# Exawind/hypre-mini-app

Measured on AMD Instinct MI355X. Metric: GMRES+AMG solve GDOF/s (N_global*iterations/t_solve; iterations/sec in iterations_per_s), 512^3 Laplacian, higher is better.
Workload: dtype f64

## Files before the change

### hypre-mini-app_amd/csrc/amg_solve.cpp

```cpp
#include <algorithm>
#include <cmath>

#include "amg.hpp"
#include "kernels.hpp"
#include "profile.hpp"
#include "solvers.hpp"

namespace mi {

bool &zero_guess_hint() {
  static bool hint = false;
  return hint;
}

static int g_zero_skip = -1;
int zero_skip_mode() {
  if (g_zero_skip < 0) {
    const char *e = getenv("MI_HYPRE_GS_ZERO_SKIP");
    g_zero_skip = e ? std::max(0, std::min(3, atoi(e))) : 3;
  }
  return g_zero_skip;
}
void set_zero_skip_mode(int mode) { g_zero_skip = std::max(0, std::min(3, mode)); }

// ... 523 lines not shown
  AmgLevel &L0 = L[0];
  const bool permuted = !L0.perm.empty();
  if (permuted)
    k::gather(f, L0.d_perm.p, L0.f.p, L0.n, s);
  else
    k::copy(f, L0.f.p, L0.n, s);
  if (zero_guess) {
    if (!zero_cycle_ignores_u(0)) k::fill(L0.u.p, L0.n, 0.0, s);
  } else if (permuted)
    k::gather(e, L0.d_perm.p, L0.u.p, L0.n, s);
  else
    k::copy(e, L0.u.p, L0.n, s);
  cycle(0, zero_guess);
  if (permuted)
    k::scatter_set(e, L0.d_perm.p, L0.u.p, L0.n, s);
  else
    k::copy(L0.u.p, e, L0.n, s);
}

void BoomerAMG::solve(ParCSR &A, ParVector &b, ParVector &x) {
  if (!is_setup) setup(A);
  if (!L.empty() && source_matrix && L[0].A == source_matrix && L[0].A->assembly_stamp != source_stamp)
    fail(1, "BoomerAMGSolve: the values of the matrix changed (IJMatrix update round) after this solver was set up on it "
            "and its first level is that matrix itself; call HYPRE_BoomerAMGSetup again");
  MI_REQUIRE(x.ncomp == b.ncomp, "BoomerAMGSolve: b and x differ in their number of components");
  MI_REQUIRE(x.n == L[0].n && b.n == L[0].n, "BoomerAMGSolve: vector size does not match the matrix");
  Comm &comm = my_comm();
  hipStream_t s = ctx().stream;
  AmgLevel &L0 = L[0];
  const bool permuted = !L0.perm.empty();
  const int n = L0.n, nc = b.ncomp;
  int it = 0;
  double rel = 0.0, bn = 0.0;
  if (p.tol > 0.0) bn = std::sqrt(par_dot_host(comm, b.all(), b.all(), b.len(), s));
  const bool zero_first = zero_guess_hint();
  zero_guess_hint() = false;
  while (it < p.max_iter) {
    const bool zero = zero_first && it == 0;
    for (int c = 0; c < nc; c++) {
      const double *bc = b.all() + (size_t)c * (size_t)n;
      double *xc = x.all() + (size_t)c * (size_t)n;
      if (it == 0 || nc > 1) {
        if (permuted)
          k::gather(bc, L0.d_perm.p, L0.f.p, n, s);
        else
          k::copy(bc, L0.f.p, n, s);
      }
      if (zero) {
        if (!zero_cycle_ignores_u(0)) k::fill(L0.u.p, n, 0.0, s);
      } else if (permuted)
        k::gather(xc, L0.d_perm.p, L0.u.p, n, s);
      else
        k::copy(xc, L0.u.p, n, s);
      cycle(0, zero);
      if (permuted)
        k::scatter_set(xc, L0.d_perm.p, L0.u.p, n, s);
      else
        k::copy(L0.u.p, xc, n, s);
    }
    it++;
    if (p.tol > 0.0) {
      double rr = 0.0;
      for (int c = 0; c < nc; c++) {
        const size_t o = (size_t)c * (size_t)n;
        A.matvec(comm, -1.0, x.all() + o, 1.0, b.all() + o, L0.tmp.p, s);
        rr += par_dot_host(comm, L0.tmp.p, L0.tmp.p, n, s);
      }
      const double rn = std::sqrt(rr);
      rel = (bn > 0.0) ? rn / bn : rn;
      if (p.print_level > 1 && comm.rank == 0) printf("    BoomerAMG cycle %3d   ||r||/||b|| = %e\n", it, rel);
      if (rel <= p.tol) break;
    }
  }
  num_iterations = it;
  final_rel_res = rel;
}

}
```

### hypre-mini-app_amd/csrc/capi.cpp

```cpp
#include <limits>
#include <algorithm>
#include <cmath>
#include <cstring>
#include <thread>

#include "HYPRE_mi_ext.h"
#include "_hypre_parcsr_ls.h"
#include "ij_assembly.hpp"
#include "kernels.hpp"
#include "profile.hpp"
#include "solvers.hpp"
#include "amg_setup_internal.hpp"

using namespace mi;

namespace {

int g_error_flag = 0;
std::string g_last_error;

int record_error(int code, const std::string &msg) {
  g_error_flag |= code;
  g_last_error = msg;
  fprintf(stderr, "mi_hypre error (%d): %s\n", code, msg.c_str());
// ... 1832 lines not shown
  API_END
}
HYPRE_Int HYPRE_MI_GetCounter(const char *name, long long *value) {
  API_BEGIN
  const std::string n(name ? name : "");
  if (n == "pool_cached_bytes" || n == "pool_hits" || n == "pool_misses") {
    long long cb = 0, h = 0, m = 0;
    dev_pool_stats(&cb, &h, &m);
    *value = n == "pool_cached_bytes" ? cb : n == "pool_hits" ? h : m;
    return 0;
  }
  if (n.rfind("arena_", 0) == 0) {
    long long mp = 0, iu = 0, pm = 0, pu = 0;
    dev_arena_stats(&mp, &iu, &pm, &pu);
    if (n == "arena_mapped_bytes") *value = mp;
    else if (n == "arena_in_use_bytes") *value = iu;
    else if (n == "arena_peak_mapped_bytes") *value = pm;
    else if (n == "arena_peak_in_use_bytes") *value = pu;
    else fail(HYPRE_ERROR_ARG, "GetCounter: unknown counter " + n);
    return 0;
  }
  if (n == "ij_device_assemblies")
    *value = ij::counters().device_assemblies;
  else if (n == "ij_value_updates")
    *value = ij::counters().value_updates;
  else if (n == "ij_device_value_updates")
    *value = ij::counters().device_value_updates;
  else if (n == "ij_update_kernels_us" || n == "ij_update_dictionary_us" || n == "ij_update_mirror_us")
    *value = (long long)(1e6 * (n == "ij_update_kernels_us" ? ij::counters().t_update_kernels
                                : n == "ij_update_dictionary_us" ? ij::counters().t_update_dict : ij::counters().t_update_mirror));
  else if (n == "ij_entries_fetched_to_host")
    *value = ij::counters().entries_fetched;
  else if (n == "ij_host_mirror_bytes")
    *value = ij::counters().host_mirror_bytes;
  else if (n == "ij_device_sort_lds_capacity")
    *value = ij::SORT_LDS_CAP;
  else if (n == "ij_last_kernels_us" || n == "ij_last_mirror_us" || n == "ij_last_format_us")
    *value = (long long)(1e6 * (n == "ij_last_kernels_us" ? ij::counters().t_kernels
                                : n == "ij_last_mirror_us" ? ij::counters().t_mirror : ij::counters().t_format));
  else if (n == "matvec_overlapped")
    *value = ctx().n_matvec_overlapped;
  else if (n == "gs_overlapped")
    *value = ctx().n_gs_overlapped;
  else if (n == "gs_in_order")
    *value = ctx().n_gs_in_order;
  else if (n == "allreduce")
    *value = ctx().n_allreduce;
  else if (n == "halo_exchange")
    *value = ctx().n_halo_exchange;
  else if (n == "allgather")
    *value = ctx().n_allgather;
  else if (n == "value_storage_row_mapped")
    *value = ctx().n_value_row_mapped;
  else if (setup_reuse_counter(n.c_str()) >= 0)
    *value = setup_reuse_counter(n.c_str());
  else if (dist_setup_counter(n.c_str()) >= 0)
    *value = dist_setup_counter(n.c_str());
  else
    fail(HYPRE_ERROR_ARG, "GetCounter: unknown counter " + n);
  API_END
}
HYPRE_Int HYPRE_MI_SetZeroGuessMode(HYPRE_Int mode) {
  API_BEGIN
  if (mode < 0 || mode > 3) fail(HYPRE_ERROR_ARG, "SetZeroGuessMode: 0..3");
  set_zero_skip_mode(mode);
  API_END
}
HYPRE_Int HYPRE_MI_BoomerAMGPoisonWorkVectors(HYPRE_Solver solver) {
  API_BEGIN
  BoomerAMG &a = AMG(solver)->amg;
  const double nan = std::numeric_limits<double>::quiet_NaN();
  hipStream_t s = ctx().stream;
  for (BoomerAMG *h = &a; h; h = h->tail.get())
    for (AmgLevel &Lv : h->L) {
      if (Lv.u.p && Lv.n) k::fill(Lv.u.p, Lv.n, nan, s);
      if (Lv.tmp.p && Lv.n) k::fill(Lv.tmp.p, Lv.n, nan, s);
      if (Lv.snap.p && Lv.n) k::fill(Lv.snap.p, Lv.n, nan, s);
    }
  MI_HIP(hipStreamSynchronize(s));
  API_END
}
HYPRE_Int HYPRE_MI_TileScheduleCheck(HYPRE_Int n, const HYPRE_BigInt *row_ptr, HYPRE_Int row_cap, HYPRE_Int tile_entries,
                                     HYPRE_Int *ntiles, HYPRE_Int *mismatch) {
  API_BEGIN
  ensure_init();
  MI_REQUIRE(n >= 0 && row_ptr && mismatch, "TileScheduleCheck: arguments");
  MI_REQUIRE(tile_entries == k::SPMV_TILE || tile_entries == k::SPMV_TILE_WIDE, "TileScheduleCheck: tile_entries is 2048 or 4096");
  static_assert(sizeof(HYPRE_BigInt) == sizeof(long long), "row pointer width");
  bool aligned_h = true, aligned_d = true;
  const std::vector<int> host = k::build_row_blocks((int)n, reinterpret_cast<const int64_t *>(row_ptr), &aligned_h, (int)row_cap,
                                                    (int)tile_entries);
  DVec<long long> ia((size_t)n + 1);
  MI_HIP(hipMemcpy(ia.p, row_ptr, ((size_t)n + 1) * sizeof(long long), hipMemcpyHostToDevice));
  DVec<int> rb;
  std::vector<int> dev;
  sk::tile_schedule_device((int)n, ia.p, (int)row_cap, (int)tile_entries, rb, dev, aligned_d, ctx().stream);
  if (ntiles) *ntiles = (HYPRE_Int)host.size() - 1;
  *mismatch = 0;
  const size_t m = std::min(host.size(), dev.size());
  for (size_t t = 0; t < m && !*mismatch; t++)
    if (host[t] != dev[t]) *mismatch = (HYPRE_Int)t + 1;
  if (!*mismatch && host.size() != dev.size()) *mismatch = (HYPRE_Int)m + 1;
  if (!*mismatch && aligned_h != aligned_d) *mismatch = (HYPRE_Int)m + 2;
  API_END
}

// ... 82 lines not shown
    unsigned long long res[3];
    differing(b, res);
    if (res[0])
      fail(HYPRE_ERROR_GENERIC, "arena self-test: a live block was overwritten: " + std::to_string(res[0]) + " of " + std::to_string(b.n) +
                                    " bytes differ, first at " + std::to_string(res[1]) + ", last at " + std::to_string(res[2]) +
                                    "; block at arena offset " + std::to_string((unsigned long long)(b.p - (unsigned char *)nullptr) & 0xffffffffffull));
    dev_free(b.p);
    cur -= b.n;
    ok++;
  };
  for (int r = 0; r < rounds; r++) {
    const unsigned long long v = rnd();
    const bool grow = live.empty() || (v & 3) != 0 || live.size() < 8;
    if (grow && live.size() < 4096) {
      const int bits = 1 + (int)(rnd() % 34);
      size_t n = (size_t)(rnd() & ((1ull << bits) - 1)) + 1;
      n = std::min<size_t>(n, (size_t)std::max<HYPRE_BigInt>(1, max_block_bytes));
      Blk b{(unsigned char *)dev_alloc(n), n, (unsigned char)(1 + (rnd() % 250))};
      for (const Blk &o : live)
        if (b.p < o.p + o.n && o.p < b.p + b.n)
          fail(HYPRE_ERROR_GENERIC, "arena self-test: the allocator handed out a block that intersects a live one (round " +
                                        std::to_string(r) + ", " + std::to_string(n) + " bytes)");
      if (getenv("MI_ARENA_TEST_OWN_FILL"))
        k::fill_bytes(b.p, n, b.tag, s);
      else
        MI_HIP(hipMemsetAsync(b.p, b.tag, n, s));
      if (getenv("MI_ARENA_TEST_VERIFY_FILL")) {
        unsigned long long res[3];
        differing(b, res);
        if (res[0])
          fail(HYPRE_ERROR_GENERIC, "arena self-test: the fill of a fresh block is incomplete: " + std::to_string(res[0]) + " of " +
                                        std::to_string(n) + " bytes, first " + std::to_string(res[1]) + ", last " + std::to_string(res[2]));
      }
      live.push_back(b);
      cur += n;
      peak = std::max(peak, cur);
    } else {
      check_and_free((size_t)(rnd() % live.size()));
    }
    if ((r & 255) == 255 && !getenv("MI_ARENA_TEST_NO_TRIM")) dev_pool_trim();
  }
  MI_HIP(hipStreamSynchronize(s));
  while (!live.empty()) check_and_free(live.size() - 1);
  dev_pool_trim();
  if (verified) *verified = ok;
  if (peak_bytes) *peak_bytes = (HYPRE_BigInt)peak;
  API_END
}
HYPRE_Int HYPRE_MI_SetValueDictionary(HYPRE_Int on) {
  API_BEGIN
  k::set_value_dictionary(on != 0);
  API_END
}
HYPRE_Int HYPRE_MI_GetGSChunk(HYPRE_Int *rows) {
  *rows = ctx().gs_chunk;
  return 0;
}
HYPRE_Int HYPRE_MI_KrylovGetResidualHistory(HYPRE_Solver solver, HYPRE_Real *norms, HYPRE_Int max_n, HYPRE_Int *n) {
  API_BEGIN
  KrylovSolver *kk = KR(solver);
  const int m = std::min<int>(max_n, (int)kk->norms.size());
  for (int i = 0; i < m; i++) norms[i] = kk->norms[(size_t)i];
  if (n) *n = (int)kk->norms.size();
  API_END
}
HYPRE_Int HYPRE_MI_KrylovGetSolveSeconds(HYPRE_Solver solver, HYPRE_Real *seconds) {
  API_BEGIN
  *seconds = KR(solver)->solve_seconds;
  API_END
}
HYPRE_Int HYPRE_MI_BoomerAMGGetNumLevels(HYPRE_Solver solver, HYPRE_Int *n) {
  API_BEGIN
  *n = (HYPRE_Int)AMG(solver)->amg.total_levels();
  API_END
}
HYPRE_Int HYPRE_MI_BoomerAMGGetOperatorComplexity(HYPRE_Solver solver, HYPRE_Real *cx) {
  API_BEGIN
  *cx = AMG(solver)->amg.operator_complexity();
  API_END
}
HYPRE_Int HYPRE_MI_BoomerAMGGetSetupSeconds(HYPRE_Solver solver, HYPRE_Real *seconds) {
  API_BEGIN
  *seconds = AMG(solver)->amg.setup_seconds;
  API_END
}
static AmgLevel &level_ref(AmgSolver *a, int level, BoomerAMG **owner = nullptr, int *local = nullptr) {
  if (level < 0 || level >= a->amg.total_levels()) fail(HYPRE_ERROR_ARG, "AMG level out of range");
  int loc = 0;
  BoomerAMG &o = a->amg.owner_of(level, loc);
  if (owner) *owner = &o;
  if (local) *local = loc;
  return o.L[(size_t)loc];
}
static const HostCSR &level_csr(AmgSolver *a, int level, int which) {
  BoomerAMG *o = nullptr;
  int loc = 0;
  AmgLevel &L = level_ref(a, level, &o, &loc);
  o->ensure_host(loc);
  switch (which) {
    case 0: return L.A->diag;
    case 1: return L.A->offd;
    case 2:
    case 3:
    case 4:
    case 5: {
      const ParCSR *M = (which == 2 || which == 4) ? L.Pm.get() : L.Rm.get();
// ... 507 lines not shown
```

### hypre-mini-app_amd/csrc/krylov.cpp

```cpp
#include <cmath>
#include <cstring>

#include "HYPRE_parcsr_ls.h"
#include "kernels.hpp"
#include "solvers.hpp"

extern "C" const char *HYPRE_MI_LastErrorMessage(void);

namespace mi {

void KrylovSolver::run_precond_setup(ParCSR &A, ParVector &b, ParVector &x) {
  if (!precond_setup) return;
  const int rc = precond_setup(precond_data, &A, &b, &x);
  if (rc) fail(rc, std::string("preconditioner setup failed: ") + HYPRE_MI_LastErrorMessage());
}


void KrylovSolver::apply_precond(ParCSR &A, ParVector &rhs, ParVector &out) {
  hipStream_t s = ctx().stream;
  if (precond_solve) {
    k::fill(out.all(), out.len(), 0.0, s);
    zero_guess_hint() = true;
    precond_solve(precond_data, &A, &rhs, &out);
    zero_guess_hint() = false;
  } else {
    k::copy(rhs.all(), out.all(), out.len(), s);
  }
}

void KrylovSolver::matvec_all(ParCSR &A, double alpha, const double *x, double beta, const double *b, double *y, int nloc,
                              int ncomp, int prof) {
  Comm &comm = current_comm();
  hipStream_t s = ctx().stream;
  for (int c = 0; c < ncomp; c++) {
    const size_t o = (size_t)c * (size_t)nloc;
    A.matvec(comm, alpha, x + o, beta, b ? b + o : nullptr, y + o, s, prof);
  }
}

BoomerAMG *KrylovSolver::amg_in_level_order(ParCSR &A, int n) const {
  static const bool enabled = !(getenv("MI_HYPRE_GMRES_PERMUTED") && atoi(getenv("MI_HYPRE_GMRES_PERMUTED")) == 0);
  if (!enabled || !precond_data) return nullptr;
  if (precond_solve != reinterpret_cast<ParSolverFcn>(&HYPRE_BoomerAMGSolve)) return nullptr;
  SolverBase *sb = static_cast<SolverBase *>(precond_data);
  if (sb->kind != SolverBase::K_AMG) return nullptr;
  BoomerAMG &amg = static_cast<AmgSolver *>(sb)->amg;
  if (!amg.is_setup || amg.p.max_iter != 1 || amg.p.tol != 0.0 || amg.L.empty()) return nullptr;
  AmgLevel &L0 = amg.L[0];
  if (L0.perm.empty() || L0.A == &A || L0.n != n || !L0.A->on_device) return nullptr;
  if (amg.source_matrix != &A || amg.source_stamp != A.assembly_stamp) return nullptr;
  return &amg;
}

BoomerAMG *KrylovSolver::enter_level_order(ParCSR &A_in, ParVector &b_in, ParVector &x_in, ParCSR *&A, ParVector *&b,
                                           ParVector *&x) {
  const int n = b_in.n, nc = b_in.ncomp;
  BoomerAMG *amg = amg_in_level_order(A_in, n);
  A = &A_in;
  b = &b_in;
  x = &x_in;
  if (!amg) return nullptr;
  hipStream_t s = ctx().stream;
  if (bp.n != n || bp.ncomp != nc) {
    bp.init(b_in.start, b_in.end, nc);
    xp.init(b_in.start, b_in.end, nc);
  }
  for (int c = 0; c < nc; c++) {
    const size_t o = (size_t)c * (size_t)n;
    k::gather(b_in.all() + o, amg->L[0].d_perm.p, bp.all() + o, n, s);
    k::gather(x_in.all() + o, amg->L[0].d_perm.p, xp.all() + o, n, s);
  }
  A = amg->L[0].A;
  b = &bp;
  x = &xp;
  return amg;
}

void KrylovSolver::leave_level_order(BoomerAMG *amg, ParVector &x_in) {
  if (!amg) return;
  for (int c = 0; c < x_in.ncomp; c++) {
    const size_t o = (size_t)c * (size_t)x_in.n;
    k::scatter_set(x_in.all() + o, amg->L[0].d_perm.p, xp.all() + o, x_in.n, ctx().stream);
  }
}

const double *KrylovSolver::precond_in_order(BoomerAMG *amg, ParCSR &A, ParVector &rhs, ParVector &out, bool need_copy) {
  if (!amg) {
    apply_precond(A, rhs, out);
    return out.all();
  }
  hipStream_t s = ctx().stream;
  AmgLevel &L0 = amg->L[0];
  const int n = L0.n, nc = rhs.ncomp;
  double *own_f = L0.f.p;
  for (int c = 0; c < nc; c++) {
    const size_t o = (size_t)c * (size_t)n;
    L0.f.p = rhs.all() + o;
    if (!amg->zero_cycle_ignores_u(0)) k::fill(L0.u.p, n, 0.0, s);
    try {
      amg->cycle(0, true);
    } catch (...) {
      L0.f.p = own_f;
      throw;
    }
    L0.f.p = own_f;
    if (nc == 1 && !need_copy) return L0.u.p;
    k::copy(L0.u.p, out.all() + o, n, s);
  }
  return out.all();
}

void GmresSolver::setup(ParCSR &A, ParVector &b, ParVector &x) {
  ensure_init();
  MI_REQUIRE(b.ncomp == x.ncomp, "GMRES: b and x differ in their number of components");
  r.init(b.start, b.end, b.ncomp);
  w.init(b.start, b.end, b.ncomp);
  if (!p.empty() && (p[0]->n != b.n || p[0]->ncomp != b.ncomp || p[0]->start != b.start)) p.clear();
  if (!z.empty() && (z[0]->n != b.n || z[0]->ncomp != b.ncomp || z[0]->start != b.start)) z.clear();
  run_precond_setup(A, b, x);
}

int GmresSolver::solve(ParCSR &A_in, ParVector &b_in, ParVector &x_in) {
  TraceRange trace_solve(flexible ? "mi_hypre FlexGMRESSolve" : (ortho ? "mi_hypre COGMRESSolve" : "mi_hypre GMRESSolve"));
  ensure_init();
  Ctx &c = ctx();
  Comm &comm = current_comm();
  hipStream_t s = c.stream;
  const double t_start = wall_time();
  const int nloc = b_in.n, nc = b_in.ncomp;
  const int n = nloc * nc;
  MI_REQUIRE(x_in.ncomp == nc && x_in.n == nloc, "GMRES: b and x differ in size");
  const int kd = k_dim < 1 ? 1 : k_dim;
  MI_REQUIRE(kd + 2 <= (ortho > 1 ? 120 : 250), "GMRES: k_dim too large for the device scalar slots");
  MI_REQUIRE(ortho >= 0 && ortho <= 2, "GMRES: orthogonalisation must be 0 (MGS), 1 or 2 (classical passes)");
  if (r.n != nloc || r.ncomp != nc) setup(A_in, b_in, x_in);
  const double epsmac = 1.e-16;
  auto basis = [&](int i) -> ParVector & {
    while ((int)p.size() <= i) {
      std::unique_ptr<ParVector> v(new ParVector());
      v->init(b_in.start, b_in.end, nc);
      p.push_back(std::move(v));
    }
    return *p[(size_t)i];
  };
  auto zvec = [&](int i) -> ParVector & {
    while ((int)z.size() <= i) {
      std::unique_ptr<ParVector> v(new ParVector());
      v->init(b_in.start, b_in.end, nc);
      z.push_back(std::move(v));
    }
    return *z[(size_t)i];
  };
  std::vector<double> cs((size_t)kd + 1, 0.0), sn((size_t)kd + 1, 0.0), rs((size_t)kd + 1, 0.0);
  std::vector<std::vector<double>> hh((size_t)kd + 1, std::vector<double>((size_t)kd, 0.0));
  double *slots = c.red_out.p;

  ParCSR *Ap;
  ParVector *bq, *xq;
  BoomerAMG *amg = enter_level_order(A_in, b_in, x_in, Ap, bq, xq);
  ParCSR &A = *Ap;
  ParVector &b = *bq;
  ParVector &x = *xq;
  auto precond = [&](ParVector &rhs, ParVector &out, bool need_copy) -> const double * {
    return precond_in_order(amg, A, rhs, out, need_copy);
  };

  auto mv = [&](double alpha, const double *xv, double beta, const double *bv, double *yv) {
    matvec_all(A, alpha, xv, beta, bv, yv, nloc, nc, k::PROF_SPMV_L0);
  };
  static const bool poll = !(getenv("MI_HYPRE_GMRES_POLL") && atoi(getenv("MI_HYPRE_GMRES_POLL")) == 0);
  auto fetch_column = [&](const double *norm_slot, double *vec, int count) {
    if (!poll || count > 255) {
      k::scale_inv_sqrt_dev(norm_slot, vec, n, s);
      MI_HIP(hipMemcpyAsync(c.h_pinned, slots, (size_t)count * sizeof(double), hipMemcpyDeviceToHost, s));
      MI_HIP(hipStreamSynchronize(s));
      return;
    }
    const unsigned long long seq = ++c.post_seq;
    k::scale_inv_sqrt_post(norm_slot, vec, n, slots, count, c.h_pinned + 256, c.h_post_flag, seq, s);
    const double t0 = wall_time();
    unsigned spins = 0;
    while (__atomic_load_n(c.h_post_flag, __ATOMIC_ACQUIRE) != seq) {
      if ((++spins & 0xffffu) == 0 && wall_time() - t0 > 30.0) {
        MI_HIP(hipStreamSynchronize(s));
        if (__atomic_load_n(c.h_post_flag, __ATOMIC_ACQUIRE) != seq) fail(1, "GMRES: the Hessenberg column was not posted");
        break;
      }
    }
    memcpy(c.h_pinned, c.h_pinned + 256, (size_t)count * sizeof(double));
  };
  ParVector &p0 = basis(0);
  mv(-1.0, x.all(), 1.0, b.all(), p0.data());
  const double b_norm = std::sqrt(par_dot_host(comm, b.all(), b.all(), n, s));
  double r_norm = std::sqrt(par_dot_host(comm, p0.data(), p0.data(), n, s));
  const double r_norm_0 = r_norm;
  const double den = (b_norm > 0.0) ? b_norm : r_norm;
  const double eps = std::max(atol, tol * den);
  int iter = 0;
  converged = false;
  norms.clear();
  norms.push_back(r_norm);
  const bool chatty = print_level > 1 && comm.rank == 0;
  bool nan_seen = (b_norm != b_norm) || (r_norm != r_norm);
  if (nan_seen && comm.rank == 0 && print_level > 0)
    printf("ERROR detected by mi_hypre GMRES: NaN in the right-hand side, the initial guess or the operator\n");
  if (chatty) {
    printf("=============================================\n\n");
    printf("Iters     resid.norm     conv.rate  rel.res.norm\n");
    printf("-----    ------------    ---------- ------------\n");
  }

  while (iter < max_iter && !nan_seen) {
    rs[0] = r_norm;
    if (r_norm == 0.0) {
      converged = true;
      break;
    }
    if (r_norm <= eps && iter >= min_iter) {
      mv(-1.0, x.all(), 1.0, b.all(), r.data());
      r_norm = std::sqrt(par_dot_host(comm, r.data(), r.data(), n, s));
      if (r_norm <= eps) {
        converged = true;
        break;
      }
      if (chatty) printf("false convergence 1\n");
    }
    k::scale(1.0 / r_norm, basis(0).data(), n, s);
    int i = 0;
    while (i < kd && iter < max_iter) {
      i++;
      iter++;
      ParVector &pi = basis(i);
      ParVector &pim1 = basis(i - 1);
      ParVector &dir = flexible ? zvec(i - 1) : r;
      const double *mp;
      {
        TraceRange tr("precond (BoomerAMG cycle)");
        mp = precond(pim1, dir, flexible);
      }
      mv(1.0, mp, 0.0, nullptr, pi.data());
      TraceRange trace_ortho("Gram-Schmidt + Givens");
      if (ortho == 0) {
        par_dot(comm, basis(0).data(), pi.data(), n, slots, s);
        for (int j = 1; j <= i; j++) {
          k::axpy_dot(slots + j - 1, -1.0, basis(j - 1).data(), pi.data(), j < i ? basis(j).data() : nullptr, n,
                      slots + j, s);
          if (comm.size > 1) comm.allreduce_dev(slots + j, 1, CommDType::F64, CommOp::SUM, s), c.n_allreduce++;
        }
        fetch_column(slots + i, pi.data(), i + 1);
        for (int j = 0; j < i; j++) hh[(size_t)j][(size_t)i - 1] = c.h_pinned[j];
      } else {
        std::vector<const double *> vecs((size_t)i);
        for (int j = 0; j < i; j++) vecs[(size_t)j] = basis(j).data();
        for (int q = 0; q < ortho; q++) {
          double *cs_dev = slots + 128 * q;
          k::mass_dot(vecs.data(), i, pi.data(), n, cs_dev, s);
          if (comm.size > 1) comm.allreduce_dev(cs_dev, (size_t)i, CommDType::F64, CommOp::SUM, s), c.n_allreduce++;
          k::mass_axpy(vecs.data(), i, cs_dev, -1.0, pi.data(), n, s);
        }
        double *nrm = (ortho == 1) ? slots + i : slots + 128 + i;
        par_dot(comm, pi.data(), pi.data(), n, nrm, s);
        fetch_column(nrm, pi.data(), 128 * (ortho - 1) + i + 1);
        for (int j = 0; j < i; j++) {
          double hsum = c.h_pinned[j];
          if (ortho > 1) hsum += c.h_pinned[128 + j];
          hh[(size_t)j][(size_t)i - 1] = hsum;
        }
        c.h_pinned[i] = c.h_pinned[128 * (ortho - 1) + i];
      }
      const double t = std::sqrt(c.h_pinned[i] > 0.0 ? c.h_pinned[i] : 0.0);
      hh[(size_t)i][(size_t)i - 1] = t;
      for (int j = 1; j < i; j++) {
        const double tt = hh[(size_t)j - 1][(size_t)i - 1];
        hh[(size_t)j - 1][(size_t)i - 1] = sn[(size_t)j - 1] * hh[(size_t)j][(size_t)i - 1] + cs[(size_t)j - 1] * tt;
        hh[(size_t)j][(size_t)i - 1] = -sn[(size_t)j - 1] * tt + cs[(size_t)j - 1] * hh[(size_t)j][(size_t)i - 1];
      }
      double gamma = std::sqrt(hh[(size_t)i - 1][(size_t)i - 1] * hh[(size_t)i - 1][(size_t)i - 1] +
                               hh[(size_t)i][(size_t)i - 1] * hh[(size_t)i][(size_t)i - 1]);
      if (gamma == 0.0) gamma = epsmac;
      cs[(size_t)i - 1] = hh[(size_t)i - 1][(size_t)i - 1] / gamma;
      sn[(size_t)i - 1] = hh[(size_t)i][(size_t)i - 1] / gamma;
      rs[(size_t)i] = -hh[(size_t)i][(size_t)i - 1] * rs[(size_t)i - 1];
      rs[(size_t)i] /= gamma;
      rs[(size_t)i - 1] = cs[(size_t)i - 1] * rs[(size_t)i - 1];
      hh[(size_t)i - 1][(size_t)i - 1] =
          sn[(size_t)i - 1] * hh[(size_t)i][(size_t)i - 1] + cs[(size_t)i - 1] * hh[(size_t)i - 1][(size_t)i - 1];
      const double prev = r_norm;
      r_norm = std::fabs(rs[(size_t)i]);
      norms.push_back(r_norm);
      if (chatty)
        printf("% 5d    %e    %f   %e\n", iter, r_norm, prev > 0 ? r_norm / prev : 0.0,
               b_norm > 0 ? r_norm / b_norm : r_norm);
      if (r_norm != r_norm) {
        nan_seen = true;
        break;
      }
      if (r_norm <= eps && iter >= min_iter) break;
    }
    if (nan_seen) break;
    std::vector<double> y(rs.begin(), rs.begin() + i);
    y[(size_t)i - 1] = y[(size_t)i - 1] / hh[(size_t)i - 1][(size_t)i - 1];
    for (int kk = i - 2; kk >= 0; kk--) {
      double t = 0.0;
      for (int j = kk + 1; j < i; j++) t -= hh[(size_t)kk][(size_t)j] * y[(size_t)j];
      t += y[(size_t)kk];
      y[(size_t)kk] = t / hh[(size_t)kk][(size_t)kk];
    }
    if (flexible) {
      for (int j = i - 1; j >= 0; j--) k::axpy(y[(size_t)j], zvec(j).data(), x.all(), n, s);
    } else {
      {
        std::vector<const double *> vp((size_t)i);
        std::vector<double> cf((size_t)i);
        for (int j = i - 1, q = 0; j >= 0; j--, q++) {
          vp[(size_t)q] = basis(j).data();
          cf[(size_t)q] = y[(size_t)j];
        }
        k::lin_comb(vp.data(), cf.data(), i, true, w.data(), n, s);
      }
      const double *mw = precond(w, r, false);
      k::axpy(1.0, mw, x.all(), n, s);
    }
    if (r_norm <= eps && iter >= min_iter) {
      mv(-1.0, x.all(), 1.0, b.all(), r.data());
      r_norm = std::sqrt(par_dot_host(comm, r.data(), r.data(), n, s));
      if (r_norm <= eps) {
        converged = true;
        break;
      }
      if (chatty) printf("false convergence 2\n");
      k::copy(r.data(), basis(0).data(), n, s);
      i = 0;
    }
    if (flexible) {
      if (i) {
        mv(-1.0, x.all(), 1.0, b.all(), basis(0).data());
        r_norm = std::sqrt(par_dot_host(comm, basis(0).data(), basis(0).data(), n, s));
      }
      continue;
    }
    for (int j = i; j > 0; j--) {
      rs[(size_t)j - 1] = -sn[(size_t)j - 1] * rs[(size_t)j];
      rs[(size_t)j] = cs[(size_t)j - 1] * rs[(size_t)j];
    }
    if (i) {
      std::vector<const double *> vp;
      std::vector<double> cf;
      for (int j = i; j > 0; j--) {
        vp.push_back(basis(j).data());
        cf.push_back(rs[(size_t)j]);
      }
      k::lin_comb(vp.data(), cf.data(), (int)vp.size(), true, basis(i).data(), n, s);
      const double *v0[2] = {basis(0).data(), basis(i).data()};
      const double c0[2] = {rs[0], 1.0};
      k::lin_comb(v0, c0, 2, true, basis(0).data(), n, s);
    }
  }
  leave_level_order(amg, x_in);
  MI_HIP(hipStreamSynchronize(s));
  num_iterations = iter;
  rel_residual_norm = (b_norm > 0.0) ? r_norm / b_norm : r_norm;
  solve_seconds = wall_time() - t_start;
// ... 208 lines not shown
```

### hypre-mini-app_amd/csrc/mi_internal.hpp

```cpp
#pragma once

#include <hip/hip_runtime.h>

#include <cstdint>
#include <cstdio>
#include <cstdlib>
#include <functional>
#include <memory>
#include <stdexcept>
#include <string>
#include <type_traits>
#include <vector>

namespace mi {

using gidx = long long;

struct Error : std::runtime_error {
  int code;
  Error(int c, const std::string &m) : std::runtime_error(m), code(c) {}
};

[[noreturn]] inline void fail(int code, const std::string &msg) { throw Error(code, msg); }

// ... 195 lines not shown
  virtual ~Comm() {}
  virtual const char *name() const = 0;
  virtual void allreduce_dev(void *buf, size_t count, CommDType t, CommOp op, hipStream_t s) = 0;
  virtual void exchange_dev(const std::vector<PeerBuf> &sends, const std::vector<PeerBuf> &recvs, hipStream_t s) = 0;
  virtual void allgather_dev(const void *send, void *recv, size_t bytes_per_rank, hipStream_t s) = 0;
  virtual void allreduce_host(void *buf, size_t count, CommDType t, CommOp op);
  virtual void allgather_host(const void *send, void *recv, size_t bytes_per_rank);
  virtual void exchange_host_fixed(const std::vector<PeerBuf> &sends, const std::vector<PeerBuf> &recvs);
  void exchange_host(const std::vector<int> &peers_send, const std::vector<std::vector<char>> &send,
                     std::vector<int> &peers_recv, std::vector<std::vector<char>> &recv);
  void allgatherv_host(const void *mine, size_t bytes, std::vector<size_t> &offs, std::vector<char> &out);
  virtual bool host_transport() const { return false; }
  void barrier();
};

std::unique_ptr<Comm> make_self_comm();
std::unique_ptr<Comm> make_rccl_comm(const void *unique_id, int rank, int size);
void rccl_get_unique_id(void *out128);

struct CommCallbacks {
  void *ctx;
  void (*allreduce)(void *ctx, void *buf, size_t count, int dtype, int op);
  void (*allgather)(void *ctx, const void *send, void *recv, size_t bytes_per_rank);
  void (*exchange)(void *ctx, int nsend, const int *send_peers, void *const *send_ptrs, const size_t *send_bytes,
                   int nrecv, const int *recv_peers, void *const *recv_ptrs, const size_t *recv_bytes);
};
std::unique_ptr<Comm> make_callback_comm(const CommCallbacks &cb, int rank, int size);
std::unique_ptr<Comm> make_ipc_exchange_comm(std::unique_ptr<Comm> &inner, size_t slot_bytes);
bool comm_check_transport_error(Comm &c, hipStream_t s);
int comm_transport_verdict(Comm &c, hipStream_t s);
std::unique_ptr<Comm> make_comm_from_env();

struct KernelTimer;

struct Ctx {
  bool inited = false;
  int device = 0;
  hipStream_t stream = nullptr;
  hipStream_t comm_stream = nullptr;
  hipEvent_t ev_packed = nullptr, ev_halo = nullptr;
  std::unique_ptr<Comm> comm;
  DVec<double> red_partials;
  DVec<double> red_out;
  DVec<unsigned> red_ticket;
  double *h_pinned = nullptr;
  unsigned long long *h_post_flag = nullptr;
  unsigned long long post_seq = 0;
  int gs_chunk = 8;
  int verbose = 0;
  KernelTimer *timer = nullptr;
  long long n_matvec_overlapped = 0, n_gs_overlapped = 0, n_gs_in_order = 0;
  long long n_allreduce = 0, n_halo_exchange = 0, n_allgather = 0;
  long long n_value_row_mapped = 0;
};
Ctx &ctx();
void ensure_init();
void zero_on_stream(void *p, size_t bytes);
Comm &current_comm();

struct TraceRange {
  explicit TraceRange(const char *name);
  ~TraceRange();
  TraceRange(const TraceRange &) = delete;
  TraceRange &operator=(const TraceRange &) = delete;
  bool on = false;
};

void parallel_for(int64_t n, const std::function<void(int64_t, int64_t, int)> &fn, int max_threads = 0);
int host_threads();
double wall_time();

}
```

### hypre-mini-app_amd/csrc/solvers.hpp

```cpp
#pragma once
#include "amg.hpp"

namespace mi {

struct SolverBase {
  enum Kind { K_GMRES, K_BICGSTAB, K_PCG, K_AMG, K_ILU, K_FSAI } kind;
  explicit SolverBase(Kind k) : kind(k) {}
  virtual ~SolverBase() {}
};

typedef int (*ParSolverFcn)(void *, void *, void *, void *);

struct AmgSolver : SolverBase {
  BoomerAMG amg;
  AmgSolver() : SolverBase(K_AMG) {}
};

struct KrylovSolver : SolverBase {
  double tol = 1e-6, atol = 0.0;
  int max_iter = 1000, min_iter = 0, k_dim = 5, print_level = 0, logging = 0;
  ParSolverFcn precond_solve = nullptr, precond_setup = nullptr;
  void run_precond_setup(ParCSR &A, ParVector &b, ParVector &x);
  void *precond_data = nullptr;
  int num_iterations = 0;
  double rel_residual_norm = 0.0;
  bool converged = false;
  std::vector<double> norms;
  double solve_seconds = 0.0;
  explicit KrylovSolver(Kind k) : SolverBase(k) {}
  void apply_precond(ParCSR &A, ParVector &rhs, ParVector &out);
  void matvec_all(ParCSR &A, double alpha, const double *x, double beta, const double *b, double *y, int nloc, int ncomp,
                  int prof);
  BoomerAMG *amg_in_level_order(ParCSR &A, int n) const;
  ParVector bp, xp;
  BoomerAMG *enter_level_order(ParCSR &A_in, ParVector &b_in, ParVector &x_in, ParCSR *&A, ParVector *&b, ParVector *&x);
  void leave_level_order(BoomerAMG *amg, ParVector &x_in);
  const double *precond_in_order(BoomerAMG *amg, ParCSR &A, ParVector &rhs, ParVector &out, bool need_copy);
};

struct GmresSolver : KrylovSolver {
  std::vector<std::unique_ptr<ParVector>> p;
  bool flexible = false;
  int ortho = 0;
  std::vector<std::unique_ptr<ParVector>> z;
  ParVector r, w;
  GmresSolver() : KrylovSolver(K_GMRES) {}
  void setup(ParCSR &A, ParVector &b, ParVector &x);
  int solve(ParCSR &A, ParVector &b, ParVector &x);
};

struct BicgstabSolver : KrylovSolver {
  ParVector r0, r, pv, v, q, sv, t;
  BicgstabSolver() : KrylovSolver(K_BICGSTAB) {}
  void setup(ParCSR &A, ParVector &b, ParVector &x);
  int solve(ParCSR &A, ParVector &b, ParVector &x);
};

struct PcgSolver : KrylovSolver {
  ParVector r, pv, sv;
  int two_norm = 0;
  PcgSolver() : KrylovSolver(K_PCG) {}
  void setup(ParCSR &A, ParVector &b, ParVector &x);
  int solve(ParCSR &A, ParVector &b, ParVector &x);
};

struct IluSolver : SolverBase {
  int ilu_type = 0, level_of_fill = 0, max_iter = 20, print_level = 0, tri_solve = 1, lower_it = 5, upper_it = 5;
  double tol = 1e-7;
  int iter_type = 0, iter_option = 0, iter_max_iter = 100;
  double iter_tol = 1e-3;
  int iter_sweeps = 0;
  double iter_correction = -1.0, iter_residual = -1.0;
  std::vector<double> iter_corr_hist, iter_res_hist;
  bool is_setup = false, levels_built = false;
  int n = 0;
  sk::DCsr LU;
  DVec<long long> dpos;
  DVec<int> order_l, order_u;
  std::vector<int> lptr, uptr;
  DVec<double> y, t, r, z;
  DVec<double> rall;
  int num_iterations = 0;
  double final_rel_res = 0.0;
  IluSolver() : SolverBase(K_ILU) {}
  void setup(ParCSR &A, Comm &comm);
  void iterative_factor(Comm &comm, long long row0);
  void apply(const double *rhs, double *out);
  int solve(ParCSR &A, ParVector &b, ParVector &x);
};

struct FsaiSolver : SolverBase {
// ... 33 lines not shown
```

### hypre-mini-app_amd/mi_hypre.py

```python
import ctypes as C
import os

import numpy as np

_HERE = os.path.dirname(os.path.abspath(__file__))
LIB_PATH = os.environ.get("MI_HYPRE_LIB") or os.path.join(_HERE, "libmi_hypre.so")

HYPRE_PARCSR = 5555
HYPRE_MEMORY_DEVICE = 1
HYPRE_EXEC_DEVICE = 1
HYPRE_ERROR_GENERIC = 1
HYPRE_ERROR_CONV = 256

c_big = C.c_longlong
c_int = C.c_int
c_dbl = C.c_double
vp = C.c_void_p

PROF_SPMV_L0, PROF_RELAX_L0, PROF_DOT, PROF_AXPY = 0, 1, 2, 3
PROF_LEVELS = 16
PROF_LVL_RESID, PROF_LVL_RELAX, PROF_LVL_RESTRICT, PROF_LVL_PROLONG = 4, 4 + 16, 4 + 32, 4 + 48
PROF_LVL_RELAX0 = 4 + 64

ALLREDUCE_FN = C.CFUNCTYPE(None, vp, vp, C.c_size_t, c_int, c_int)
# ... 707 lines not shown


def laplace3d(nx, ny, nz, stencil, ilower, iupper):
    nnz = c_big()
    rows, cols, vals, rhs = vp(), vp(), vp(), vp()
    call("HYPRE_MI_Laplace3D", nx, ny, nz, stencil, c_big(ilower), c_big(iupper), C.byref(nnz), C.byref(rows),
         C.byref(cols), C.byref(vals), C.byref(rhs))
    return dict(nnz=nnz.value, rows=rows.value, cols=cols.value, vals=vals.value, rhs=rhs.value,
                nloc=iupper - ilower + 1)


def laplace3d_free(g):
    for k in ("rows", "cols", "vals", "rhs"):
        if g.get(k):
            lib().HYPRE_MI_Free(vp(g[k]))
            g[k] = None


def laplace3d_device(nx, ny, nz, stencil, ilower, iupper):
    nnz = c_big()
    rows, cols, vals, rhs = vp(), vp(), vp(), vp()
    call("HYPRE_MI_Laplace3DDevice", nx, ny, nz, stencil, c_big(ilower), c_big(iupper), C.byref(nnz), C.byref(rows),
         C.byref(cols), C.byref(vals), C.byref(rhs))
    return dict(nnz=nnz.value, rows=rows.value, cols=cols.value, vals=vals.value, rhs=rhs.value,
                nloc=iupper - ilower + 1)


def laplace3d_device_free(g):
    lib().HYPRE_MI_FreeDevice.argtypes = [vp]
    lib().HYPRE_MI_FreeDevice.restype = None
    for k in ("rows", "cols", "vals", "rhs"):
        if g.get(k):
            lib().HYPRE_MI_FreeDevice(vp(g[k]))
            g[k] = None


def counter(name):
    v = C.c_longlong()
    call("HYPRE_MI_GetCounter", name.encode(), C.byref(v))
    return v.value


def assembly_stamp(A):
    par = A.par if hasattr(A, "par") else A
    v = C.c_ulonglong()
    call("HYPRE_MI_ParCSRGetAssemblyStamp", par, C.byref(v))
    return v.value


def set_value_dictionary(on):
    call("HYPRE_MI_SetValueDictionary", 1 if on else 0)


def parcsr_value_kind(A):
    par = A.par if hasattr(A, "par") else A
    v = c_int()
    call("HYPRE_MI_ParCSRGetValueKind", par, C.byref(v))
    return v.value


def parcsr_csr(A, which):
    par = A.par if hasattr(A, "par") else A
    nr, nc, nnz = c_int(), c_int(), c_big()
    call("HYPRE_MI_ParCSRGetCSRSize", par, which, C.byref(nr), C.byref(nc), C.byref(nnz))
    ia = np.zeros(nr.value + 1, dtype=np.int64)
    ja = np.zeros(max(nnz.value, 1), dtype=np.int32)
    a = np.zeros(max(nnz.value, 1), dtype=np.float64)
    call("HYPRE_MI_ParCSRGetCSR", par, which, ia, ja, a)
    return ia, ja[: nnz.value], a[: nnz.value], (nr.value, nc.value)


def parcsr_colmap(A):
    par = A.par if hasattr(A, "par") else A
    nr, nc, nnz = c_int(), c_int(), c_big()
    call("HYPRE_MI_ParCSRGetCSRSize", par, 1, C.byref(nr), C.byref(nc), C.byref(nnz))
    cm = np.zeros(max(nc.value, 1), dtype=np.int64)
    call("HYPRE_MI_ParCSRGetColMapOffd", par, cm)
    return cm[: nc.value]


def build_laplace_system(nx, ny, nz, stencil=7, rank=0, size=1):
    N = nx * ny * nz
    ilower, iupper = row_partition(N, size, rank)
    A = IJMatrix(ilower, iupper)
    g = laplace3d(nx, ny, nz, stencil, ilower, iupper)
    A.set_values_ptr(g["nnz"], g["rows"], g["cols"], g["vals"])
    A.assemble()
    rhs = np.ctypeslib.as_array(C.cast(g["rhs"], C.POINTER(c_dbl)), shape=(g["nloc"],)).copy()
    laplace3d_free(g)
    b = IJVector(ilower, iupper, rhs)
    x = IJVector(ilower, iupper)
    x.fill(0.0)
    return A, b, x, rhs


def profile_enable(pid, capacity=4096):
    call("HYPRE_MI_ProfileEnable", pid, capacity)


def profile_reset():
    call("HYPRE_MI_ProfileReset")


def profile_kernel_name(pid):
    buf = C.create_string_buffer(128)
    call("HYPRE_MI_ProfileKernelName", pid, buf, 128)
# ... 287 lines not shown
```

### include/HYPRE_mi_ext.h

```cpp
#ifndef HYPRE_MI_EXT_HEADER
#define HYPRE_MI_EXT_HEADER
#include "HYPRE_parcsr_ls.h"
#include "HYPRE_IJ_mv.h"
#ifdef __cplusplus
extern "C" {
#endif

#define HYPRE_MI_UNIQUE_ID_BYTES 128
HYPRE_Int HYPRE_MI_CommGetUniqueId(void *id128);
HYPRE_Int HYPRE_MI_CommInitRCCL(const void *id128, HYPRE_Int rank, HYPRE_Int size);
HYPRE_Int HYPRE_MI_CommInitFromEnv(void);
typedef void (*HYPRE_MI_AllreduceFn)(void *ctx, void *buf, size_t count, int dtype ,
                                     int op );
typedef void (*HYPRE_MI_AllgatherFn)(void *ctx, const void *send, void *recv, size_t bytes_per_rank);
typedef void (*HYPRE_MI_ExchangeFn)(void *ctx, int nsend, const int *send_peers, void *const *send_ptrs,
                                    const size_t *send_bytes, int nrecv, const int *recv_peers, void *const *recv_ptrs,
                                    const size_t *recv_bytes);
HYPRE_Int HYPRE_MI_CommInitCallbacks(void *ctx, HYPRE_MI_AllreduceFn ar, HYPRE_MI_AllgatherFn ag,
                                     HYPRE_MI_ExchangeFn ex, HYPRE_Int rank, HYPRE_Int size);
HYPRE_Int HYPRE_MI_CommEnablePeerStoreExchange(HYPRE_BigInt slot_bytes);
HYPRE_Int HYPRE_MI_CommCheck(void);
HYPRE_Int HYPRE_MI_CommAllreduceDevice(HYPRE_Real *dev_buf, HYPRE_Int count);
HYPRE_Int HYPRE_MI_CommExchangeDevice(HYPRE_Int nsend, const HYPRE_Int *send_peers, void *const *send_ptrs,
                                      const size_t *send_bytes, HYPRE_Int nrecv, const HYPRE_Int *recv_peers,
                                      void *const *recv_ptrs, const size_t *recv_bytes);
HYPRE_Int HYPRE_MI_CommName(char *name, HYPRE_Int max_len);
HYPRE_Int HYPRE_MI_CommSelfTestRCCL(void);
HYPRE_Int HYPRE_MI_CommFinalize(void);
HYPRE_Int HYPRE_MI_CommRank(HYPRE_Int *rank);
HYPRE_Int HYPRE_MI_CommSize(HYPRE_Int *size);
HYPRE_Int HYPRE_MI_CommBarrier(void);
HYPRE_Int HYPRE_MI_CommAllreduce(void *buf, size_t count, int dtype, int op);

HYPRE_Int HYPRE_MI_IJMatrixAssembleHostOnly(HYPRE_IJMatrix matrix);
HYPRE_Int HYPRE_MI_BoomerAMGSetupHostOnly(HYPRE_Solver solver, HYPRE_ParCSRMatrix A);
HYPRE_Int HYPRE_MI_ParCSRGetHaloPlan(HYPRE_ParCSRMatrix A, HYPRE_Int *nsend_peers, HYPRE_Int *send_peers,
                                     HYPRE_Int *send_starts, HYPRE_Int *send_map, HYPRE_Int *nrecv_peers,
                                     HYPRE_Int *recv_peers, HYPRE_Int *recv_starts);

HYPRE_Int HYPRE_MI_ParCSRGetCSRSize(HYPRE_ParCSRMatrix A, HYPRE_Int which, HYPRE_Int *nrows, HYPRE_Int *ncols,
                                    HYPRE_BigInt *nnz);
HYPRE_Int HYPRE_MI_ParCSRGetCSR(HYPRE_ParCSRMatrix A, HYPRE_Int which, HYPRE_BigInt *ia, HYPRE_Int *ja, HYPRE_Complex *a);
HYPRE_Int HYPRE_MI_ParCSRGetColMapOffd(HYPRE_ParCSRMatrix A, HYPRE_BigInt *col_map_offd);
HYPRE_Int HYPRE_MI_ParCSRGetAssemblyStamp(HYPRE_ParCSRMatrix A, unsigned long long *stamp);
HYPRE_Int HYPRE_MI_ParCSRGetValueKind(HYPRE_ParCSRMatrix A, HYPRE_Int *kind);

HYPRE_Int HYPRE_MI_GetStream(void **hip_stream);
HYPRE_Int HYPRE_MI_StreamSynchronize(void);
HYPRE_Int HYPRE_MI_SetGSChunk(HYPRE_Int rows_per_chunk);
HYPRE_Int HYPRE_MI_GetGSChunk(HYPRE_Int *rows_per_chunk);
HYPRE_Int HYPRE_MI_SetZeroGuessMode(HYPRE_Int mode);
HYPRE_Int HYPRE_MI_BoomerAMGPoisonWorkVectors(HYPRE_Solver solver);
HYPRE_Int HYPRE_MI_TileScheduleCheck(HYPRE_Int n, const HYPRE_BigInt *row_ptr, HYPRE_Int row_cap, HYPRE_Int tile_entries,
                                     HYPRE_Int *ntiles, HYPRE_Int *mismatch);
HYPRE_Int HYPRE_MI_VectorKernelOp(HYPRE_Int op, HYPRE_Int m, HYPRE_ParVector *vecs, const HYPRE_Real *coef,
                                  HYPRE_Real scale, HYPRE_ParVector w, HYPRE_ParVector xd, HYPRE_Int init,
                                  HYPRE_Real *out);
HYPRE_Int HYPRE_MI_ArenaSelfTest(HYPRE_Int seed, HYPRE_Int rounds, HYPRE_BigInt max_block_bytes, HYPRE_BigInt *verified,
                                 HYPRE_BigInt *peak_bytes);
HYPRE_Int HYPRE_MI_SetValueDictionary(HYPRE_Int on);
HYPRE_Int HYPRE_MI_GetCounter(const char *name, long long *value);
HYPRE_Int HYPRE_MI_CheckBlockRowPointers(HYPRE_BigInt nrows, const HYPRE_BigInt *row_ptr);

HYPRE_Int HYPRE_MI_KrylovGetResidualHistory(HYPRE_Solver solver, HYPRE_Real *norms, HYPRE_Int max_n, HYPRE_Int *n);
HYPRE_Int HYPRE_MI_KrylovGetSolveSeconds(HYPRE_Solver solver, HYPRE_Real *seconds);

HYPRE_Int HYPRE_MI_CSRDeviceOp(HYPRE_Int op, HYPRE_Int a_nrows, HYPRE_Int a_ncols, const HYPRE_BigInt *a_ia,
                               const HYPRE_Int *a_ja, const HYPRE_Complex *a_a, HYPRE_Int b_nrows, HYPRE_Int b_ncols,
                               const HYPRE_BigInt *b_ia, const HYPRE_Int *b_ja, const HYPRE_Complex *b_a,
                               const HYPRE_Int *perm, const HYPRE_Int *colpos, HYPRE_Int *c_nrows, HYPRE_Int *c_ncols,
                               HYPRE_BigInt **c_ia, HYPRE_Int **c_ja, HYPRE_Complex **c_a);

HYPRE_Int HYPRE_MI_CSRReuseOp(HYPRE_Int op, HYPRE_Int a_nrows, HYPRE_Int a_ncols, const HYPRE_BigInt *a_ia, const HYPRE_Int *a_ja,
                              const HYPRE_Complex *a_a, HYPRE_Int b_nrows, HYPRE_Int b_ncols, const HYPRE_BigInt *b_ia,
                              const HYPRE_Int *b_ja, const HYPRE_Complex *b_a, const HYPRE_Int *rowmap, const HYPRE_Int *colmap,
                              HYPRE_Int lanes, HYPRE_Int c_nrows, HYPRE_Int c_ncols, const HYPRE_BigInt *c_ia,
                              const HYPRE_Int *c_ja, HYPRE_Complex *c_a, HYPRE_Int *bad_row);

HYPRE_Int HYPRE_MI_MMInterpOp(HYPRE_Int type, HYPRE_Int n, const HYPRE_BigInt *a_ia, const HYPRE_Int *a_ja,
                              const HYPRE_Complex *a_a, const HYPRE_BigInt *s_ia, const HYPRE_Int *s_ja, const HYPRE_Int *cf,
                              HYPRE_Real trunc_factor, HYPRE_Int pmax, HYPRE_Int lanes, HYPRE_Int *p_ncols,
                              HYPRE_BigInt **p_ia, HYPRE_Int **p_ja, HYPRE_Complex **p_a, HYPRE_Int *bad_row);

HYPRE_Int HYPRE_MI_AIRRestrictionOp(HYPRE_Int on_host, HYPRE_Int n, const HYPRE_BigInt *a_ia, const HYPRE_Int *a_ja,
                                    const HYPRE_Complex *a_a, const HYPRE_Int *cf, HYPRE_Real strong_threshold_r,
                                    HYPRE_Real filter_threshold_r, HYPRE_Int *r_nrows, HYPRE_BigInt **r_ia, HYPRE_Int **r_ja,
                                    HYPRE_Complex **r_a, HYPRE_Int info[8]);
HYPRE_Int HYPRE_MI_FSAIAdaptiveOp(HYPRE_Int on_host, HYPRE_Int n, const HYPRE_BigInt *b_ia, const HYPRE_Int *b_ja,
                                  const HYPRE_Complex *b_a, HYPRE_Int max_steps, HYPRE_Int max_step_size,
                                  HYPRE_Real kap_tolerance, HYPRE_Int table_slots, HYPRE_BigInt **g_ia, HYPRE_Int **g_ja,
                                  HYPRE_Complex **g_a, HYPRE_Int info[8]);
HYPRE_Int HYPRE_MI_FSAIGetSetupInfo(HYPRE_Solver solver, HYPRE_Int out[8]);
HYPRE_Int HYPRE_MI_OnePointInterpOp(HYPRE_Int on_host, HYPRE_Int n, const HYPRE_BigInt *a_ia, const HYPRE_Int *a_ja,
                                    const HYPRE_Complex *a_a, const HYPRE_BigInt *s_ia, const HYPRE_Int *s_ja,
                                    const HYPRE_Int *cf, HYPRE_Int *p_ncols, HYPRE_BigInt **p_ia, HYPRE_Int **p_ja,
                                    HYPRE_Complex **p_a);
HYPRE_Int HYPRE_MI_BoomerAMGGetRestrictionInfo(HYPRE_Solver solver, HYPRE_Int level, HYPRE_Int out[4]);

HYPRE_Int HYPRE_MI_BoomerAMGSetSetupReuse(HYPRE_Solver solver, HYPRE_Int mode);
HYPRE_Int HYPRE_MI_BoomerAMGGetSetupKind(HYPRE_Solver solver, HYPRE_Int *kind, HYPRE_Int *reason);
const char *HYPRE_MI_SetupReuseReasonText(HYPRE_Int reason);

HYPRE_Int HYPRE_MI_BoomerAMGGetNumLevels(HYPRE_Solver solver, HYPRE_Int *num_levels);
HYPRE_Int HYPRE_MI_BoomerAMGGetOperatorComplexity(HYPRE_Solver solver, HYPRE_Real *cx);
HYPRE_Int HYPRE_MI_BoomerAMGGetSetupSeconds(HYPRE_Solver solver, HYPRE_Real *seconds);
HYPRE_Int HYPRE_MI_BoomerAMGGetLevelCSRSize(HYPRE_Solver solver, HYPRE_Int level, HYPRE_Int which, HYPRE_Int *nrows,
                                            HYPRE_Int *ncols, HYPRE_BigInt *nnz);
HYPRE_Int HYPRE_MI_BoomerAMGGetLevelCSR(HYPRE_Solver solver, HYPRE_Int level, HYPRE_Int which, HYPRE_BigInt *ia,
                                        HYPRE_Int *ja, HYPRE_Complex *a);
HYPRE_Int HYPRE_MI_BoomerAMGGetLevelCF(HYPRE_Solver solver, HYPRE_Int level, HYPRE_Int *cf);
HYPRE_Int HYPRE_MI_BoomerAMGGetLevelNorms(HYPRE_Solver solver, HYPRE_Int level, HYPRE_Real *diag, HYPRE_Real *l1gs,
                                          HYPRE_Real *l1jac);
HYPRE_Int HYPRE_MI_BoomerAMGSetValueStorage(HYPRE_Solver solver, HYPRE_Int mode, HYPRE_Int first_level);
// ... 56 lines not shown
```

Before: 3.766.

## Keep preconditioned GMRES directions to avoid extra AMG cycle at restart update

Right-preconditioned GMRES now stores each preconditioned direction M^{-1}v_i, by default and when allocation succeeds, in the flexible-GMRES z vectors. The solution update becomes a linear combination of those stored vectors, so the final preconditioner application per restart cycle is no longer needed. For single-component runs it swaps the AMG output buffer pointer rather than copying. The trade is extra device memory for up to kdim vectors, with a fallback that handles allocation failure collectively across ranks. Counters and API hooks are added for testing.

After: 3.919, median of 6. 1.04x the previous value.

```diff
diff --git a/hypre-mini-app_amd/csrc/amg_solve.cpp b/hypre-mini-app_amd/csrc/amg_solve.cpp
--- a/hypre-mini-app_amd/csrc/amg_solve.cpp
+++ b/hypre-mini-app_amd/csrc/amg_solve.cpp
@@ -599,6 +599,7 @@
         k::gather(xc, L0.d_perm.p, L0.u.p, n, s);
       else
         k::copy(xc, L0.u.p, n, s);
+      if (ctx().krylov_precond_depth > 0) ctx().n_precond_cycles++;
       cycle(0, zero);
       if (permuted)
         k::scatter_set(xc, L0.d_perm.p, L0.u.p, n, s);
diff --git a/hypre-mini-app_amd/csrc/capi.cpp b/hypre-mini-app_amd/csrc/capi.cpp
--- a/hypre-mini-app_amd/csrc/capi.cpp
+++ b/hypre-mini-app_amd/csrc/capi.cpp
@@ -1908,6 +1908,10 @@
     *value = ctx().n_allgather;
   else if (n == "value_storage_row_mapped")
     *value = ctx().n_value_row_mapped;
+  else if (n == "precond_cycles")
+    *value = ctx().n_precond_cycles;
+  else if (n == "gmres_direction_vectors")
+    *value = ctx().n_gmres_z_allocated;
   else if (setup_reuse_counter(n.c_str()) >= 0)
     *value = setup_reuse_counter(n.c_str());
   else if (dist_setup_counter(n.c_str()) >= 0)
@@ -2096,6 +2100,16 @@
   k::set_value_dictionary(on != 0);
   API_END
 }
+HYPRE_Int HYPRE_MI_SetGmresKeepDirections(HYPRE_Int on) {
+  API_BEGIN
+  gmres_keep_directions() = on != 0;
+  API_END
+}
+HYPRE_Int HYPRE_MI_TestGmresDirectionAllocFailsAt(HYPRE_Int at) {
+  API_BEGIN
+  gmres_keep_fail_at() = at < 0 ? -1 : (int)at;
+  API_END
+}
 HYPRE_Int HYPRE_MI_GetGSChunk(HYPRE_Int *rows) {
   *rows = ctx().gs_chunk;
   return 0;
diff --git a/hypre-mini-app_amd/csrc/krylov.cpp b/hypre-mini-app_amd/csrc/krylov.cpp
--- a/hypre-mini-app_amd/csrc/krylov.cpp
+++ b/hypre-mini-app_amd/csrc/krylov.cpp
@@ -15,12 +15,29 @@
   if (rc) fail(rc, std::string("preconditioner setup failed: ") + HYPRE_MI_LastErrorMessage());
 }
 
+
+namespace {
+struct PrecondScope {
+  PrecondScope() { ctx().krylov_precond_depth++; }
+  ~PrecondScope() { ctx().krylov_precond_depth--; }
+};
+}
+
+bool &gmres_keep_directions() {
+  static bool on = !(getenv("MI_HYPRE_GMRES_KEEP_DIRECTIONS") && atoi(getenv("MI_HYPRE_GMRES_KEEP_DIRECTIONS")) == 0);
+  return on;
+}
+int &gmres_keep_fail_at() {
+  static int at = -1;
+  return at;
+}
 
 void KrylovSolver::apply_precond(ParCSR &A, ParVector &rhs, ParVector &out) {
   hipStream_t s = ctx().stream;
   if (precond_solve) {
     k::fill(out.all(), out.len(), 0.0, s);
     zero_guess_hint() = true;
+    PrecondScope scope;
     precond_solve(precond_data, &A, &rhs, &out);
     zero_guess_hint() = false;
   } else {
@@ -97,6 +114,7 @@
     const size_t o = (size_t)c * (size_t)n;
     L0.f.p = rhs.all() + o;
     if (!amg->zero_cycle_ignores_u(0)) k::fill(L0.u.p, n, 0.0, s);
+    ctx().n_precond_cycles++;
     try {
       amg->cycle(0, true);
     } catch (...) {
@@ -148,8 +166,28 @@
       std::unique_ptr<ParVector> v(new ParVector());
       v->init(b_in.start, b_in.end, nc);
       z.push_back(std::move(v));
+      c.n_gmres_z_allocated++;
     }
     return *z[(size_t)i];
+  };
+  auto try_zvec = [&](int i) -> ParVector * {
+    if ((int)z.size() > i) return z[(size_t)i].get();
+    int ok = !(gmres_keep_fail_at() >= 0 && i >= gmres_keep_fail_at());
+    if (ok) {
+      try {
+        zvec(i);
+      } catch (const Error &e) {
+        if (e.code != 2) throw;
+        ok = 0;
+      }
+    }
+    if (comm.size > 1) {
+      int all = ok;
+      comm.allreduce_host(&all, 1, CommDType::I32, CommOp::MIN);
+      if (ok && !all) z.pop_back();
+      ok = all;
+    }
+    return ok ? z[(size_t)i].get() : nullptr;
   };
   std::vector<double> cs((size_t)kd + 1, 0.0), sn((size_t)kd + 1, 0.0), rs((size_t)kd + 1, 0.0);
   std::vector<std::vector<double>> hh((size_t)kd + 1, std::vector<double>((size_t)kd, 0.0));
@@ -164,6 +202,13 @@
   auto precond = [&](ParVector &rhs, ParVector &out, bool need_copy) -> const double * {
     return precond_in_order(amg, A, rhs, out, need_copy);
   };
+  bool keep = amg && !flexible && gmres_keep_directions();
+  if (comm.size > 1 && !flexible && gmres_keep_directions() &&
+      precond_solve == reinterpret_cast<ParSolverFcn>(&HYPRE_BoomerAMGSolve)) {
+    int all = keep ? 1 : 0;
+    comm.allreduce_host(&all, 1, CommDType::I32, CommOp::MIN);
+    keep = all != 0;
+  }
 
   auto mv = [&](double alpha, const double *xv, double beta, const double *bv, double *yv) {
     matvec_all(A, alpha, xv, beta, bv, yv, nloc, nc, k::PROF_SPMV_L0);
@@ -227,17 +272,22 @@
     }
     k::scale(1.0 / r_norm, basis(0).data(), n, s);
     int i = 0;
+    bool kept = keep;
     while (i < kd && iter < max_iter) {
       i++;
       iter++;
       ParVector &pi = basis(i);
       ParVector &pim1 = basis(i - 1);
-      ParVector &dir = flexible ? zvec(i - 1) : r;
+      ParVector *zk = kept ? try_zvec(i - 1) : nullptr;
+      if (kept && !zk) keep = kept = false;
+      const bool adopt = zk && nc == 1 && amg->L[0].u.n == zk->d.n;
+      ParVector &dir = flexible ? zvec(i - 1) : (zk ? *zk : r);
       const double *mp;
       {
         TraceRange tr("precond (BoomerAMG cycle)");
-        mp = precond(pim1, dir, flexible);
-      }
+        mp = precond(pim1, dir, flexible || (zk && !adopt));
+      }
+      if (adopt) std::swap(amg->L[0].u.p, zk->d.p);
       mv(1.0, mp, 0.0, nullptr, pi.data());
       TraceRange trace_ortho("Gram-Schmidt + Givens");
       if (ortho == 0) {
@@ -308,6 +358,14 @@
     }
     if (flexible) {
       for (int j = i - 1; j >= 0; j--) k::axpy(y[(size_t)j], zvec(j).data(), x.all(), n, s);
+    } else if (kept) {
+      std::vector<const double *> vp((size_t)i);
+      std::vector<double> cf((size_t)i);
+      for (int j = i - 1, q = 0; j >= 0; j--, q++) {
+        vp[(size_t)q] = zvec(j).data();
+        cf[(size_t)q] = y[(size_t)j];
+      }
+      k::lin_comb(vp.data(), cf.data(), i, false, x.all(), n, s);
     } else {
       {
         std::vector<const double *> vp((size_t)i);
diff --git a/hypre-mini-app_amd/csrc/mi_internal.hpp b/hypre-mini-app_amd/csrc/mi_internal.hpp
--- a/hypre-mini-app_amd/csrc/mi_internal.hpp
+++ b/hypre-mini-app_amd/csrc/mi_internal.hpp
@@ -271,6 +271,8 @@
   long long n_matvec_overlapped = 0, n_gs_overlapped = 0, n_gs_in_order = 0;
   long long n_allreduce = 0, n_halo_exchange = 0, n_allgather = 0;
   long long n_value_row_mapped = 0;
+  long long n_precond_cycles = 0, n_gmres_z_allocated = 0;
+  int krylov_precond_depth = 0;
 };
 Ctx &ctx();
 void ensure_init();
diff --git a/hypre-mini-app_amd/csrc/solvers.hpp b/hypre-mini-app_amd/csrc/solvers.hpp
--- a/hypre-mini-app_amd/csrc/solvers.hpp
+++ b/hypre-mini-app_amd/csrc/solvers.hpp
@@ -37,6 +37,9 @@
   void leave_level_order(BoomerAMG *amg, ParVector &x_in);
   const double *precond_in_order(BoomerAMG *amg, ParCSR &A, ParVector &rhs, ParVector &out, bool need_copy);
 };
+
+bool &gmres_keep_directions();
+int &gmres_keep_fail_at();
 
 struct GmresSolver : KrylovSolver {
   std::vector<std::unique_ptr<ParVector>> p;
diff --git a/hypre-mini-app_amd/mi_hypre.py b/hypre-mini-app_amd/mi_hypre.py
--- a/hypre-mini-app_amd/mi_hypre.py
+++ b/hypre-mini-app_amd/mi_hypre.py
@@ -783,6 +783,10 @@
     call("HYPRE_MI_SetValueDictionary", 1 if on else 0)
 
 
+def set_gmres_keep_directions(on):
+    call("HYPRE_MI_SetGmresKeepDirections", 1 if on else 0)
+
+
 def parcsr_value_kind(A):
     par = A.par if hasattr(A, "par") else A
     v = c_int()
diff --git a/include/HYPRE_mi_ext.h b/include/HYPRE_mi_ext.h
--- a/include/HYPRE_mi_ext.h
+++ b/include/HYPRE_mi_ext.h
@@ -59,6 +59,8 @@
 HYPRE_Int HYPRE_MI_ArenaSelfTest(HYPRE_Int seed, HYPRE_Int rounds, HYPRE_BigInt max_block_bytes, HYPRE_BigInt *verified,
                                  HYPRE_BigInt *peak_bytes);
 HYPRE_Int HYPRE_MI_SetValueDictionary(HYPRE_Int on);
+HYPRE_Int HYPRE_MI_SetGmresKeepDirections(HYPRE_Int on);
+HYPRE_Int HYPRE_MI_TestGmresDirectionAllocFailsAt(HYPRE_Int at);
 HYPRE_Int HYPRE_MI_GetCounter(const char *name, long long *value);
 HYPRE_Int HYPRE_MI_CheckBlockRowPointers(HYPRE_BigInt nrows, const HYPRE_BigInt *row_ptr);
 
```
